# TuringLang/AdvancedHMC.jl

Hardware: AMD Instinct MI355X
Metric: leapfrog-steps/sec (whole node) at n_chains x D (higher is better)
Workload: dtype f64

## Files before the change

### advancedhmc.jl_amd/csrc/ahmc_device.hpp

```cpp
#pragma once

#include <hip/hip_runtime.h>
#include <stdint.h>

namespace ahmc {

enum : uint32_t { RNG_MOMENTUM = 0, RNG_TRANSITION = 1, RNG_JITTER = 2, RNG_FINDEPS = 3 };
constexpr uint32_t COUPLED_CHAIN = 0xFFFFFFFFu;

struct Philox4 {
  uint32_t v[4];
};

__device__ __forceinline__ Philox4 philox4x32_10(uint32_t c0, uint32_t c1, uint32_t c2, uint32_t c3,
                                                 uint32_t k0, uint32_t k1) {
  constexpr uint32_t M0 = 0xD2511F53u, M1 = 0xCD9E8D57u, W0 = 0x9E3779B9u, W1 = 0xBB67AE85u;
#pragma unroll
  for (int round = 0; round < 10; ++round) {
    uint32_t hi0 = __umulhi(M0, c0), lo0 = M0 * c0;
    uint32_t hi1 = __umulhi(M1, c2), lo1 = M1 * c2;
    uint32_t n0 = hi1 ^ c1 ^ k0, n2 = hi0 ^ c3 ^ k1;
    c0 = n0; c1 = lo1; c2 = n2; c3 = lo0;
    k0 += W0; k1 += W1;
  }
// ... 130 lines not shown
  q = q * t;
  return __builtin_ldexp(__builtin_fma(tj, q, tj), k >> 6);
  }
  {
  const double xh = x < -1100.0 ? -1100.0 : x;
  const double dn = __builtin_rint(xh * C(0x3ff71547652b82feULL));
  double t = __builtin_fma(dn, C(0xbfe62e42fefa39efULL), xh);
  t = __builtin_fma(dn, C(0xbc7abc9e3b39803fULL), t);
  double q = __builtin_fma(t, C(0x3e5ade156a5dcb37ULL), C(0x3e928af3fca7ab0cULL));
  q = fma3(t, q, C(0x3ec71dee623fde64ULL));
  q = fma3(t, q, C(0x3efa01997c89e6b0ULL));
  q = fma3(t, q, C(0x3f2a01a014761f6eULL));
  q = fma3(t, q, C(0x3f56c16c1852b7b0ULL));
  q = fma3(t, q, C(0x3f81111111122322ULL));
  q = fma3(t, q, C(0x3fa55555555502a1ULL));
  q = fma3(t, q, C(0x3fc5555555555511ULL));
  q = fma3(t, q, C(0x3fe000000000000bULL));
  q = __builtin_fma(t, q, 1.0);
  q = __builtin_fma(t, q, 1.0);
  double z = __builtin_ldexp(q, (int)dn);
  return z;
  }
}
template <bool UNIFORM>
__device__ __forceinline__ float leaf_weight_exp(float x) { return exp(x); }

template <class T, bool UNIFORM>
__device__ __forceinline__ T alpha_from_logweight(T lw) {
  const T w = leaf_weight_exp<UNIFORM>(lw > T(0) ? T(0) : lw);
  return w >= T(1) ? T(1) : w;
}

template <int LA, int LB>
__device__ __forceinline__ double leaf_weight_exp_pair(double x, bool odd) {
  constexpr auto C = [](unsigned long long bits) { return __builtin_bit_cast(double, bits); };
  const double xc = x < -1100.0 ? -1100.0 : x;
  const double dk = __builtin_rint(xc * 92.33248261689366);
  double t = __builtin_fma(dk, -0x1.62e42fef00000p-7, xc);
  t = __builtin_fma(dk, -0x1.473de6af278edp-40, t);
  const int k = (int)dk;
  const int ka = __builtin_amdgcn_readlane(k, LA), kb = __builtin_amdgcn_readlane(k, LB);
  const double tja = C(EXP2_64_BITS[ka & 63]), tjb = C(EXP2_64_BITS[kb & 63]);
  const double tj = odd ? tjb : tja;
  double q = __builtin_fma(t, 8.3333333333333332e-03, 4.1666666666666664e-02);
  q = fma3(t, q, 1.6666666666666666e-01);
  q = fma3(t, q, 0.5);
  q = fma3(t, q, 1.0);
  q = q * t;
  return __builtin_ldexp(__builtin_fma(tj, q, tj), k >> 6);
}
template <int LA, int LB>
__device__ __forceinline__ float leaf_weight_exp_pair(float x, bool) { return exp(x); }

template <class T> __device__ __forceinline__ T maxabs(T a, T b) { return fabs(a) > fabs(b) ? a : b; }

template <int CTRL> __device__ __forceinline__ int dpp_i32(int v) {
  return __builtin_amdgcn_mov_dpp(v, CTRL, 0xf, 0xf, true);
}
template <int CTRL> __device__ __forceinline__ float dpp_mov(float v) {
  return __int_as_float(dpp_i32<CTRL>(__float_as_int(v)));
}
template <int CTRL> __device__ __forceinline__ double dpp_mov(double v) {
  int lo = __double2loint(v), hi = __double2hiint(v);
  return __hiloint2double(dpp_i32<CTRL>(hi), dpp_i32<CTRL>(lo));
}
__device__ __forceinline__ float swz16(float v) {
  return __int_as_float(__builtin_amdgcn_ds_swizzle(__float_as_int(v), 0x401F));
}
__device__ __forceinline__ double swz16(double v) {
  int lo = __builtin_amdgcn_ds_swizzle(__double2loint(v), 0x401F);
  int hi = __builtin_amdgcn_ds_swizzle(__double2hiint(v), 0x401F);
  return __hiloint2double(hi, lo);
}
__device__ __forceinline__ float xor16_sum(float v) {
  auto p = __builtin_amdgcn_permlane16_swap(__float_as_int(v), __float_as_int(v), false, false);
  return __int_as_float(p[0]) + __int_as_float(p[1]);
}
__device__ __forceinline__ double xor16_sum(double v) {
  auto lo = __builtin_amdgcn_permlane16_swap(__double2loint(v), __double2loint(v), false, false);
  auto hi = __builtin_amdgcn_permlane16_swap(__double2hiint(v), __double2hiint(v), false, false);
  return __hiloint2double(hi[0], lo[0]) + __hiloint2double(hi[1], lo[1]);
}
__device__ __forceinline__ float xor32_sum(float v) {
  auto p = __builtin_amdgcn_permlane32_swap(__float_as_int(v), __float_as_int(v), false, false);
  return __int_as_float(p[0]) + __int_as_float(p[1]);
}
__device__ __forceinline__ double xor32_sum(double v) {
  auto lo = __builtin_amdgcn_permlane32_swap(__double2loint(v), __double2loint(v), false, false);
  auto hi = __builtin_amdgcn_permlane32_swap(__double2hiint(v), __double2hiint(v), false, false);
  return __hiloint2double(hi[0], lo[0]) + __hiloint2double(hi[1], lo[1]);
}

#ifndef AHMC_MFMA_REDUCE
#define AHMC_MFMA_REDUCE 0
#endif
template <class T> struct MfmaRed;
template <> struct MfmaRed<double> {
  typedef double acc_t __attribute__((ext_vector_type(4)));
  static __device__ __forceinline__ acc_t mma(double a, double b, acc_t c) { return __builtin_amdgcn_mfma_f64_16x16x4f64(a, b, c, 0, 0, 0); }
  static constexpr unsigned SEL = 8u;
  static constexpr int RA = 0, RB = 2;
};
template <> struct MfmaRed<float> {
  typedef float acc_t __attribute__((ext_vector_type(4)));
  static __device__ __forceinline__ acc_t mma(float a, float b, acc_t c) { return __builtin_amdgcn_mfma_f32_16x16x4f32(a, b, c, 0, 0, 0); }
  static constexpr unsigned SEL = 1u;
// ... 87 lines not shown
    return (__builtin_amdgcn_ballot_w64(x <= T(0)) & 3ull) != 0ull;
  }
}

template <int G, class T>
__device__ __forceinline__ void wave_allsum4(T& a, T& b, T& c, T& d) {
  static_assert(G == 16 || G == 32 || G == 64, "quad reduction needs whole 16-lane rows");
  const bool odd = (threadIdx.x & 1u) != 0, up = (threadIdx.x & 2u) != 0;
  const T x = (odd ? b : a) + dpp_mov<0xB1>(odd ? a : b);
  const T y = (odd ? d : c) + dpp_mov<0xB1>(odd ? c : d);
  T z = (up ? y : x) + dpp_mov<0x4E>(up ? x : y);
  z += dpp_mov<0x124>(z);
  z += dpp_mov<0x128>(z);
  if constexpr (G >= 32) z = xor16_sum(z);
  if constexpr (G >= 64) z = xor32_sum(z);
  a = dpp_mov<0x150>(z);
  b = dpp_mov<0x151>(z);
  c = dpp_mov<0x152>(z);
  d = dpp_mov<0x153>(z);
}

#ifndef AHMC_PAIR_RED_QUAD
#define AHMC_PAIR_RED_QUAD 1
#endif
template <class T, int Q = AHMC_PAIR_RED_QUAD>
__device__ __forceinline__ bool wave64_pair_reduce(T da, T db, T& ea, T& eb) {
  static_assert(Q >= 0 && Q <= 3, "a row has four quads");
  const bool odd = (threadIdx.x & 1u) != 0, up = (threadIdx.x & 2u) != 0;
  const T x = (odd ? db : da) + dpp_mov<0xB1>(odd ? da : db);
  const T y = (odd ? eb : ea) + dpp_mov<0xB1>(odd ? ea : eb);
  T z = (up ? y : x) + dpp_mov<0x4E>(up ? x : y);
  z += dpp_mov<0x124>(z);
  z += dpp_mov<0x128>(z);
  z = xor16_sum(z);
  z = xor32_sum(z);
  const bool le0 = (__builtin_amdgcn_ballot_w64(z <= T(0)) & 3ull) != 0ull;
  ea = dpp_mov<0x150 + 4 * Q + 2>(z);
  eb = dpp_mov<0x150 + 4 * Q + 3>(z);
  return le0;
}
template <class T>
__device__ __forceinline__ bool wave64_pair_reduce_t(T da, T db, T ea, T eb, T& z) {
  const bool odd = (threadIdx.x & 1u) != 0, up = (threadIdx.x & 2u) != 0;
  const T x = (odd ? db : da) + dpp_mov<0xB1>(odd ? da : db);
  const T y = (odd ? eb : ea) + dpp_mov<0xB1>(odd ? ea : eb);
  z = (up ? y : x) + dpp_mov<0x4E>(up ? x : y);
  z += dpp_mov<0x124>(z);
  z += dpp_mov<0x128>(z);
  z = xor16_sum(z);
  z = xor32_sum(z);
  return (__builtin_amdgcn_ballot_w64(z <= T(0)) & 3ull) != 0ull;
}

template <int G, class T, int K>
__device__ __forceinline__ void wave_allsum(T (&v)[K]) {
  static_assert(G == 1 || G == 2 || G == 4 || G == 8 || G == 16 || G == 32 || G == 64, "bad group size");
  if constexpr (G >= 16 && K == 4) {
    wave_allsum4<G>(v[0], v[1], v[2], v[3]);
    return;
  }
  if constexpr (G >= 16 && K % 2 == 0) {
#pragma unroll
    for (int k = 0; k < K; k += 2) wave_allsum2<G>(v[k], v[k + 1]);
    return;
  }
  if constexpr (G >= 2) {
#pragma unroll
    for (int k = 0; k < K; ++k) v[k] += dpp_mov<0xB1>(v[k]);
  }
  if constexpr (G >= 4) {
#pragma unroll
    for (int k = 0; k < K; ++k) v[k] += dpp_mov<0x4E>(v[k]);
  }
  if constexpr (G >= 8) {
#pragma unroll
    for (int k = 0; k < K; ++k) v[k] += dpp_mov<0x141>(v[k]);
  }
  if constexpr (G >= 16) {
#pragma unroll
    for (int k = 0; k < K; ++k) v[k] += dpp_mov<0x140>(v[k]);
  }
  if constexpr (G >= 32) {
#pragma unroll
    for (int k = 0; k < K; ++k) {
      if constexpr ((AHMC_DS_REDUCE & 1) != 0) v[k] += ds_swz<SWZ_XOR16>(v[k]); else v[k] = xor16_sum(v[k]);
    }
  }
  if constexpr (G >= 64) {
#pragma unroll
    for (int k = 0; k < K; ++k) {
      if constexpr ((AHMC_DS_REDUCE & 1) != 0) v[k] += ds_xor32(v[k]); else v[k] = xor32_sum(v[k]);
    }
  }
}
__device__ __forceinline__ double* xwave_buf() {
  __shared__ __attribute__((aligned(16))) double buf[8 * 8];
  return buf;
}

template <int G, class T, int K>
__device__ __forceinline__ void group_allsum(T (&v)[K]) {
  if constexpr (G <= 64) {
    wave_allsum<G>(v);
  } else {
    static_assert(G == 128 || G == 256 || G == 512, "bad multi-wave group size");
    static_assert(K <= 8, "at most 8 values per reduction");
// ... 327 lines not shown
#pragma unroll
  for (int e = 0; e < E; ++e) z.r[e] = leapfrog_kick(z.r[e], eh, z.g[e]);
#pragma unroll
  for (int e = 0; e < E; ++e) z.th[e] = leapfrog_drift(z.th[e], eps, minv[e], z.r[e]);
  const T part = target_eval<T, G, E, TK>(tp, z.th, z.g, lane, d0);
#pragma unroll
  for (int e = 0; e < E; ++e) z.r[e] = leapfrog_kick(z.r[e], eh, z.g[e]);
  const T kin = kinetic_partial(z.r, minv);
  return part - kin / 2;
}
template <class T>
__device__ __forceinline__ T neg_energy_sanitized(T s) { return is_finite(s) ? s : -Lim<T>::inf(); }

template <int L> __device__ __forceinline__ float readlane_t(float v) { return __int_as_float(__builtin_amdgcn_readlane(__float_as_int(v), L)); }
template <int L> __device__ __forceinline__ double readlane_t(double v) {
  return __hiloint2double(__builtin_amdgcn_readlane(__double2hiint(v), L), __builtin_amdgcn_readlane(__double2loint(v), L));
}

template <class T> struct PairLeafStats {
  T w[2], sa[2], dH[2];
  bool redo[2], div[2];
};
template <class T, bool LINW, int Q = AHMC_PAIR_RED_QUAD>
__device__ __forceinline__ void pair_leaf_stats(T z, T H0, T delta_max, T lw_limit, PairLeafStats<T>& o) {
  static_assert(Q >= 0 && Q <= 3, "a row has four quads");
  constexpr int LA = 4 * Q + 2, LB = 4 * Q + 3;
  const bool odd = (threadIdx.x & 1u) != 0;
  const T ne = neg_energy_sanitized(dpp_mov<0xEE>(z));
  const T dH = -ne - H0;
  const T lw = H0 + ne;
  T w, sa;
  if constexpr (LINW) {
    w = leaf_weight_exp_pair<LA, LB>(lw, odd);
    sa = w >= T(1) ? T(1) : w;
  } else {
    const T wa = leaf_weight_exp_pair<LA, LB>(lw > T(0) ? T(0) : lw, odd);
    sa = wa >= T(1) ? T(1) : wa;
    w = lw;
  }
  const unsigned long long m_redo = __builtin_amdgcn_ballot_w64(lw > lw_limit);
  const unsigned long long m_div = __builtin_amdgcn_ballot_w64(!(-H0 < delta_max + ne));
  o.w[0] = readlane_t<LA>(w);
  o.w[1] = readlane_t<LB>(w);
  o.sa[0] = readlane_t<LA>(sa);
  o.sa[1] = readlane_t<LB>(sa);
  o.dH[0] = readlane_t<LA>(dH);
  o.dH[1] = readlane_t<LB>(dH);
  o.redo[0] = LINW && ((m_redo >> LA) & 1ull) != 0ull;
  o.redo[1] = LINW && ((m_redo >> LB) & 1ull) != 0ull;
  o.div[0] = ((m_div >> LA) & 1ull) != 0ull;
  o.div[1] = ((m_div >> LB) & 1ull) != 0ull;
}

template <class T, int G, int E, int TK, class F>
__device__ __forceinline__ void leapfrog_step_plus2(Point<T, E>& z, const T (&minv)[E], T eps, const TargetP<T>& tp, int lane, int d0,
                                                    T (&extra)[2], F&& partials, bool use_pre = false) {
  const T eh = eps / 2;
#pragma unroll
  for (int e = 0; e < E; ++e) z.r[e] = leapfrog_kick(z.r[e], eh, z.g[e]);
#pragma unroll
  for (int e = 0; e < E; ++e) z.th[e] = leapfrog_drift(z.th[e], eps, minv[e], z.r[e]);
  T red[4];
  red[0] = target_eval<T, G, E, TK>(tp, z.th, z.g, lane, d0, use_pre);
#pragma unroll
  for (int e = 0; e < E; ++e) z.r[e] = leapfrog_kick(z.r[e], eh, z.g[e]);
  red[1] = kinetic_partial(z.r, minv);
  partials(red[2], red[3]);
  hier_publish_next<T, G, E, TK>(z, minv, eps);
  leapfrog_allsum<G, TK>(red);
  z.lp = sanitize(red[0]);
  z.lk = sanitize(-red[1] / 2);
  extra[0] = red[2];
  extra[1] = red[3];
}

template <class T, int G, int E, int TK>
__device__ __forceinline__ void fill_caches(Point<T, E>& z, const T (&minv)[E], const TargetP<T>& tp, int lane, int d0) {
  T red[2];
  red[0] = target_eval<T, G, E, TK>(tp, z.th, z.g, lane, d0);
  red[1] = kinetic_partial(z.r, minv);
  leapfrog_allsum<G, TK>(red);
  z.lp = sanitize(red[0]);
  z.lk = sanitize(-red[1] / 2);
}

template <class T, int E, bool SB = false>
__device__ __forceinline__ void load_vec(T (&v)[E], const T* __restrict__ base, int64_t off, int d0, int D, T pad) {
  constexpr int CH = (E * sizeof(T) >= 16) ? (int)(16 / sizeof(T)) : E;
  if constexpr (SB) {
    const T* sb = base + off;
    if (CH > 1 && d0 + E <= D && (reinterpret_cast<uintptr_t>(sb) % (CH * sizeof(T)) == 0)) {
      using V = T __attribute__((ext_vector_type(CH)));
      unsigned bv = (unsigned)d0 * (unsigned)sizeof(T);
      asm("; full lane" : "+v"(bv));
      const T* ptr = reinterpret_cast<const T*>(reinterpret_cast<const char*>(sb) + bv);
#pragma unroll
      for (int e = 0; e < E; e += CH) {
        V t = *reinterpret_cast<const V*>(ptr + e);
#pragma unroll
        for (int k = 0; k < CH; ++k) v[e + k] = t[k];
      }
    } else {
#pragma unroll
      for (int e = 0; e < E; ++e) {
        v[e] = pad;
        if (d0 + e < D) {
// ... 69 lines not shown
```

### advancedhmc.jl_amd/csrc/ahmc_nuts.hpp

```cpp
#pragma once

#ifndef AHMC_LEAF_PROF
#define AHMC_LEAF_PROF 0
#endif
#if AHMC_LEAF_PROF
#undef AHMC_WAVE_TIMELINE
#define AHMC_WAVE_TIMELINE 1
#define AHMC_TL_WORDS 24
#define AHMC_LP_TICK(i) { __builtin_amdgcn_sched_barrier(0); const unsigned n_ = (unsigned)__builtin_amdgcn_readfirstlane((int)(unsigned)__builtin_readcyclecounter()); __builtin_amdgcn_sched_barrier(0); lp_t[i] += n_ - lp_c; lp_c = n_; }
#define AHMC_LP_COUNT(i, n) { lp_t[i] += (unsigned)(n); }
#else
#define AHMC_LP_TICK(i)
#define AHMC_LP_COUNT(i, n)
#endif
#ifndef AHMC_WAVE_TIMELINE
#define AHMC_WAVE_TIMELINE 0
#endif
#ifndef AHMC_TL_WORDS
#define AHMC_TL_WORDS 8
#endif

#include <type_traits>

#include "ahmc_kernels.hpp"



namespace ahmc {

template <bool ON, class P>
__device__ __forceinline__ const P* args_reread() {
  if constexpr (ON) {
    auto k = __builtin_amdgcn_kernarg_segment_ptr();
    asm volatile("" : "+s"(k));
    return (const P*)k;
  } else {
    return nullptr;
  }
}
template <bool ON, class P>
__device__ __forceinline__ const P& args_at(const P& p, const P* q) {
  if constexpr (ON) return *q;
  else return p;
}

template <bool ON, class A, class P>
__device__ __forceinline__ auto adapt_block_at(const A* ak, const P* args) {
  if constexpr (ON) return (const __attribute__((address_space(4))) A*)args->adaptk;
  else return ak;
}
template <bool ON, class Q>
__device__ __forceinline__ Q* as_global(Q* q) {
  if constexpr (ON) return (Q*)(__attribute__((address_space(1))) Q*)q;
  else return q;
}

__device__ __forceinline__ int64_t wave_scalar64(int64_t x) {
  const uint32_t lo = (uint32_t)__builtin_amdgcn_readfirstlane((int)(uint32_t)x), hi = (uint32_t)__builtin_amdgcn_readfirstlane((int)(uint32_t)((uint64_t)x >> 32));
  return (int64_t)(((uint64_t)hi << 32) | lo);
}

constexpr double LINW_LIMIT = 600.0;
enum { SL_OTH_TH = 0, SL_OTH_R = 1, SL_OTH_G = 2, SL_TREE_A = 3, SL_Z0_R = 4, SL_Z0_G = 5, SL_START_R = 6 };

template <class T, int E>
struct Chunking {
  static constexpr int CH = (E * sizeof(T) >= 16) ? (int)(16 / sizeof(T)) : E;
  static constexpr int NCH = E / CH;
};

#define AHMC_AS_LDS __attribute__((address_space(3)))
#define AHMC_AS_GLB __attribute__((address_space(1)))
template <class T, int E>
struct Slots {
  AHMC_AS_LDS T* lds;
  AHMC_AS_GLB T* glb;
  int n_lds;
  unsigned lane_off;

#define AHMC_SLOT_PUT(AS)                                                                                   \
  static __device__ __forceinline__ void put(AS T* __restrict__ sb, unsigned off, const T (&v)[E]) {         \
    constexpr int CH = Chunking<T, E>::CH, NCH = Chunking<T, E>::NCH;                                       \
    if constexpr (CH > 1) {                                                                                 \
      using V = T __attribute__((ext_vector_type(CH)));                                                     \
      _Pragma("unroll") for (int c = 0; c < NCH; ++c) {                                                     \
        V t;                                                                                                \
        _Pragma("unroll") for (int k = 0; k < CH; ++k) t[k] = v[c * CH + k];                                \
        *(AS V*)(&sb[off + (unsigned)(c * 64 * CH)]) = t;                                                    \
      }                                                                                                     \
    } else {                                                                                                \
      _Pragma("unroll") for (int c = 0; c < NCH; ++c) sb[off + (unsigned)(c * 64)] = v[c];                  \
    }                                                                                                       \
  }                                                                                                         \
  static __device__ __forceinline__ void get(const AS T* __restrict__ sb, unsigned off, T (&v)[E]) {         \
    constexpr int CH = Chunking<T, E>::CH, NCH = Chunking<T, E>::NCH;                                       \
    if constexpr (CH > 1) {                                                                                 \
      using V = T __attribute__((ext_vector_type(CH)));                                                     \
      _Pragma("unroll") for (int c = 0; c < NCH; ++c) {                                                     \
        V t = *(const AS V*)(&sb[off + (unsigned)(c * 64 * CH)]);                                            \
        _Pragma("unroll") for (int k = 0; k < CH; ++k) v[c * CH + k] = t[k];                                \
      }                                                                                                     \
    } else {                                                                                                \
      _Pragma("unroll") for (int c = 0; c < NCH; ++c) v[c] = sb[off + (unsigned)(c * 64)];                  \
    }                                                                                                       \
  }
  AHMC_SLOT_PUT(AHMC_AS_LDS)
  AHMC_SLOT_PUT(AHMC_AS_GLB)
#undef AHMC_SLOT_PUT
  __device__ __forceinline__ void store(int slot, const T (&v)[E]) const {
    constexpr int SE = Chunking<T, E>::NCH * 64 * Chunking<T, E>::CH;
    if (slot < n_lds) put(lds + slot * SE, lane_off, v);
    else put(glb + (size_t)(slot - n_lds) * SE, lane_off, v);
  }
  __device__ __forceinline__ void load(int slot, T (&v)[E]) const {
    constexpr int SE = Chunking<T, E>::NCH * 64 * Chunking<T, E>::CH;
    if (slot < n_lds) get(lds + slot * SE, lane_off, v);
    else get(glb + (size_t)(slot - n_lds) * SE, lane_off, v);
  }
  __device__ __forceinline__ void store_cold(int slot, unsigned extra, const T (&v)[E]) const {
    constexpr int SE = Chunking<T, E>::NCH * 64 * Chunking<T, E>::CH;
    put(glb + (size_t)(slot - n_lds) * SE, lane_off + extra, v);
  }
  __device__ __forceinline__ void load_cold(int slot, unsigned extra, T (&v)[E]) const {
    constexpr int SE = Chunking<T, E>::NCH * 64 * Chunking<T, E>::CH;
    get(glb + (size_t)(slot - n_lds) * SE, lane_off + extra, v);
  }
};

template <class T, int G, int E, int TK, bool TEMPER = true>
__device__ __forceinline__ void leapfrog_core(Point<T, E>& z, const T (&minv)[E], T eps, const TargetP<T>& tp,
                                              const LeapfrogP<T>& lf, int lane, int d0) {
  if constexpr (TEMPER) temper(lf, z.r, 1, true, 1);
  const T eh = eps / 2;
#pragma unroll
  for (int e = 0; e < E; ++e) z.r[e] = leapfrog_kick(z.r[e], eh, z.g[e]);
#pragma unroll
  for (int e = 0; e < E; ++e) z.th[e] = leapfrog_drift(z.th[e], eps, minv[e], z.r[e]);
  (void)target_eval<T, G, E, TK>(tp, z.th, z.g, lane, d0);
#pragma unroll
  for (int e = 0; e < E; ++e) z.r[e] = leapfrog_kick(z.r[e], eh, z.g[e]);
  if constexpr (TEMPER) temper(lf, z.r, 1, false, 1);
}

template <bool WIDE>
struct DrawStreamT {
  static constexpr uint32_t PERIOD = !WIDE ? 4u : 256u;
  Rng rng;
  uint32_t k;
  Philox4 blk;
  __device__ __forceinline__ uint32_t lane_block() const {
    if constexpr (!WIDE) return 0u;
    else return threadIdx.x & 63u;
  }
  __device__ __forceinline__ void init(const Rng& r) { rng = r; k = 0; }
  __device__ __forceinline__ void resume(const Rng& r, uint32_t k0) {
    rng = r;
    k = k0;
    if (k & (PERIOD - 1u)) blk = rng.raw(RNG_TRANSITION, ((k & ~(PERIOD - 1u)) >> 2) + lane_block());
  }
  __device__ __forceinline__ uint32_t word() {
    if ((k & (PERIOD - 1u)) == 0u) blk = rng.raw(RNG_TRANSITION, (k >> 2) + lane_block());
    const uint32_t lo = (k & 1u) ? blk.v[1] : blk.v[0], hi = (k & 1u) ? blk.v[3] : blk.v[2];
    uint32_t w = (k & 2u) ? hi : lo;
    if constexpr (WIDE) {
      const uint32_t ks = (uint32_t)__builtin_amdgcn_readfirstlane((int)k);
      const int src = (int)((ks >> 2) & 63u);
      w = (uint32_t)__builtin_amdgcn_readlane((int)w, src);
    }
    ++k;
    return w;
  }
  __device__ __forceinline__ double uniform() { return ((double)word() + 0.5) * 2.3283064365386962890625e-10; }
  __device__ __forceinline__ bool boolean() { return (word() >> 31) != 0; }
  __device__ __forceinline__ double randexp() { return -log(uniform()); }
};
typedef DrawStreamT<false> DrawStream;

template <class T, int G, int E, int MODE, int TK>
__global__ __launch_bounds__((G > 256 ? G : 256), (E >= 16 ? 1 : (MODE == 2 ? (E <= 2 ? 3 : 2) : (E <= 2 ? 4 : (E <= 4 ? 3 : 2))))) void k_nuts(KP<T> p) {
  constexpr int CPW = G >= 64 ? 1 : 64 / G;
  if constexpr (G == 64 && (MODE == 0 || MODE == 3)) {
    const unsigned int wave_id = blockIdx.x * (blockDim.x >> 6) + (threadIdx.x >> 6);
    if (wave_id >= p.n_chunks) {
      const unsigned int tw = (unsigned int)__builtin_amdgcn_readfirstlane((int)(wave_id - p.n_chunks));
      const int64_t rows = (int64_t)p.tail_n_trans * p.N, row0 = (int64_t)tw * p.tail_rows;
      if (tw < p.tail_waves && row0 < rows)
        normals_rows(p, p.tail_out, p.tail_iteration, (uint32_t)RNG_MOMENTUM, row0, row0 + p.tail_rows < rows ? row0 + p.tail_rows : rows, (int)(threadIdx.x & 63));
      return;
    }
  }
#define AHMC_UNI(b) (CPW == 1 ? (__builtin_amdgcn_ballot_w64(b) != 0) : (b))
#define AHMC_ANY(b) (CPW == 1 ? (bool)(b) : (__builtin_amdgcn_ballot_w64(b) != 0))
  constexpr int NCH = Chunking<T, E>::NCH, CH = Chunking<T, E>::CH;
  constexpr int SLOT_ELEMS = NCH * 64 * CH;
  extern __shared__ __attribute__((aligned(16))) unsigned char smem[];
  const int nwaves = blockDim.x >> 6;
  const int wib = threadIdx.x >> 6;
  const int lane64 = threadIdx.x & 63;
  int lane = (int)(threadIdx.x & (G - 1));
  int gi = G >= 64 ? 0 : lane64 / G;
  int d0 = lane * E;
  const int NLEV = p.max_depth > 1 ? p.max_depth - 1 : 1;
  constexpr bool LINW = MODE == 0 || MODE == 3;
  constexpr bool GENERAL = MODE == 2;
  constexpr bool FUSE_M0 = !GENERAL && G > 64;
  constexpr bool ADAPT = MODE >= 3;
  constexpr bool UTURN_ANY = G == 64;
  constexpr bool PAIR = G == 64 && !GENERAL && UTURN_ANY && !AHMC_MFMA_REDUCE && (AHMC_DS_REDUCE & 3) == 0 &&
                        !AHMC_LEAF_PROF && !AHMC_WAVE_TIMELINE;
  const bool strict = GENERAL && p.criterion == 2;
  const int NV = strict ? 3 : 2;
  const int n_slots = NV * NLEV + NUTS_DORMANT + NUTS_CKPT;
  const int CK0 = NV * NLEV + NUTS_DORMANT;
  const int n_lds_slots = p.n_lds_levels;
  T* lds_vec = reinterpret_cast<T*>(smem) + (size_t)wib * n_lds_slots * SLOT_ELEMS;
  T* sT = reinterpret_cast<T*>(smem) + (size_t)nwaves * n_lds_slots * SLOT_ELEMS + (size_t)wib * NUTS_NSC * NLEV * CPW;
  T* sAT = reinterpret_cast<T*>(smem) + (size_t)nwaves * (n_lds_slots * SLOT_ELEMS + NUTS_NSC * NLEV * CPW) + (size_t)wib * NUTS_NAT * CPW;
  int* sIbase = reinterpret_cast<int*>(reinterpret_cast<T*>(smem) + (size_t)nwaves * (n_lds_slots * SLOT_ELEMS + (NUTS_NSC * NLEV + NUTS_NAT) * CPW));
  int* sI = sIbase + (size_t)wib * NUTS_NSI * NLEV * CPW;
  int* sAI = sIbase + (size_t)nwaves * NUTS_NSI * NLEV * CPW + (size_t)wib * NUTS_NAI * CPW;
#define A_EPSNOM sAT[0 * CPW + gi]
#define A_DAEPS sAT[1 * CPW + gi]
#define A_DAMU sAT[2 * CPW + gi]
#define A_DAXBAR sAT[3 * CPW + gi]
#define A_DAHBAR sAT[4 * CPW + gi]
#define A_DAM sAI[0 * CPW + gi]
#define A_WVN sAI[1 * CPW + gi]
#define A_CHK sAI[2 * CPW + gi]
#define S_W(lvl) sT[((0) * NLEV + (lvl)) * CPW + gi]
#define S_CK(lvl) sI[((1) * NLEV + (lvl)) * CPW + gi]
  constexpr bool TSC = G == 64 && !GENERAL;
  const int64_t wave_slot = (int64_t)blockIdx.x * nwaves + wib;
  Slots<T, E> sl;
  sl.lds = (AHMC_AS_LDS T*)lds_vec;
  sl.glb = (AHMC_AS_GLB T*)(p.scratch + wave_slot * (int64_t)(n_slots - n_lds_slots) * SLOT_ELEMS);
  sl.n_lds = n_lds_slots;
  sl.lane_off = (unsigned)lane64 * CH;
  const int DORM = NV * NLEV;
  const int NL_HOT = NLEV < 4 ? NLEV : 4;
  const int HOT_END = 2 * NL_HOT - 1;
  const int COLD_DORM = HOT_END + 2 + 2 * (NLEV > 4 ? NLEV - 4 : 0);
  auto LA = [&](int l) -> int {
    if constexpr (GENERAL) return NV * l;
    else return l == 0 ? 0 : (l < NL_HOT ? 2 * l - 1 : HOT_END + 2 + 2 * (l - 4));
  };
  auto LRF = [&](int l) -> int {
    if constexpr (GENERAL) return NV * l + 1;
    else return l == 0 ? 0 : (l < NL_HOT ? 2 * l : HOT_END + 3 + 2 * (l - 4));
  };
  auto DS = [&](int k) -> int {
    if constexpr (GENERAL) return DORM + k;
    else return k == SL_TREE_A ? HOT_END : (k == SL_OTH_R ? HOT_END + 1
                : COLD_DORM + (k == SL_OTH_TH ? 0 : k == SL_OTH_G ? 1 : k == SL_Z0_R ? 2 : k == SL_Z0_G ? 3 : 4));
  };
  const bool classic = GENERAL && p.criterion == 0;
  const bool slice = GENERAL && p.sampler == 2;

  const unsigned int chunk = G > 64 ? blockIdx.x : blockIdx.x * nwaves + wib;
  if (chunk >= p.n_chunks) return;
  const int64_t slot = (int64_t)chunk * CPW + gi;
  const int64_t c = slot < p.N ? (p.order ? (int64_t)p.order[slot] : slot) : p.N;
  int64_t cc = c < p.N ? c : 0;
  if constexpr (TSC) cc = wave_scalar64(cc);
  const int kt0 = p.redo_only ? p.redo[cc] - 1 : 0;
  bool active = c < p.N && kt0 >= 0;
  if (!AHMC_ANY(active)) return;
  T minv[E];
  load_minv<T, E, TSC>(p, cc, d0, minv);
  T th_cur[E];
  load_vec<T, E, TSC>(th_cur, p.th(), cc * p.D, d0, p.D, T(0));
  const AdaptK<T>* ak0 = ADAPT ? static_cast<const AdaptK<T>*>(p.adaptk) : nullptr;
  const AdaptK<T>* ak = ak0;
  const KP<T>*pa_ = nullptr, *pe_ = nullptr;

  auto schedule = [&](int kt2, bool& do_push, bool& do_update, bool& wv_reset, bool& dareset) {
    do_push = do_update = wv_reset = dareset = false;
    if (ak->kind == AHMC_ADAPT_STAN) {
      const int64_t si = ak->stan_i0 + kt2 + 1;
      const bool in_window = si >= ak->window_start && si <= ak->window_end;
      bool window_end = false;
      for (int k2 = 0; k2 < ak->n_splits; ++k2) window_end = window_end || ak->splits[k2] == si;
      if (in_window && ak->has_mm) { do_push = true; do_update = window_end; }
      if (window_end) { dareset = true; wv_reset = ak->has_mm != 0; }
    } else if (ak->has_mm) {
      do_push = true;
      do_update = true;
    }
    if (ak->pooled) { do_update = false; wv_reset = false; }
// ... 76 lines not shown
      bool vleft = false;
      if (!done) vleft = AHMC_UNI(ds.boolean());
      const int v = vleft ? -1 : 1;
      const bool need_swap = AHMC_UNI(!done && (vleft != cur_is_left));
      if (AHMC_ANY(need_swap)) {
        if (need_swap) {
          if (jw > 0) {
            Point<T, E> t;
            sl.load(DS(SL_OTH_TH), t.th);
            sl.load(DS(SL_OTH_R), t.r);
            sl.load(DS(SL_OTH_G), t.g);
            sl.store(DS(SL_OTH_TH), cur.th);
            sl.store(DS(SL_OTH_R), cur.r);
            sl.store(DS(SL_OTH_G), cur.g);
            copy_vec(cur.th, t.th);
            copy_vec(cur.r, t.r);
            copy_vec(cur.g, t.g);
          }
          int ti = pos_cur; pos_cur = pos_oth; pos_oth = ti;
          cur_is_left = vleft;
        }
      }
      if (strict && AHMC_ANY(!done)) {
        if (!done) sl.store(DS(SL_START_R), cur.r);
      }
      if (CKPT && jw >= CKPT_MIN_JW) {
        bool ck_save = true;
        if constexpr (CPW == 1) ck_save = AHMC_UNI(!done && pos_cur != 0);
        if (ck_save) {
          const unsigned xo = (unsigned)(((A_CHK & 1) ^ 1) * 3 * SLOT_ELEMS);
          sl.store_cold(CK0 + 0, xo, cur.th);
          sl.store_cold(CK0 + 1, xo, cur.r);
          sl.store_cold(CK0 + 2, xo, cur.g);
        }
      }
      const uint32_t nleaf = 1u << jw;
      bool alive = !done;
      bool sub_term = false;
      T A_c[E], RF_c[E];
      T w_c = 0, sa_c = 0, dh_c = 0;
      int na_c = 0, ck_c = 0;
      AHMC_LP_TICK(5)
      for (uint32_t leaf = 1; leaf <= nleaf; ++leaf) {
        if (!AHMC_ANY(alive)) break;
        AHMC_LP_COUNT(8, 1)
#if AHMC_WAVE_TIMELINE
        tl_steps += 1;
        tl_alive += (unsigned long long)__builtin_popcountll(__builtin_amdgcn_ballot_w64(alive && lane == 0));
#endif
        bool pair = false;
        if constexpr (PAIR) {
          pair = jw > 0;
          if (pair) ++leaf;
        }
        const int nm = __builtin_ctz(leaf);
        T dots_m0[2] = {0, 0}, RF_m0[E];
        if (pair) {
          if constexpr (PAIR) {
            const T es = v > 0 ? eps : -eps;
            T ea = leapfrog_step_ne_partial<T, G, E, TK>(cur, minv, es, p.tp, lane, d0);
            T r_a[E];
            copy_vec(r_a, cur.r);
            T eb = leapfrog_step_ne_partial<T, G, E, TK>(cur, minv, es, p.tp, lane, d0);
            T dots[2] = {0, 0};
#pragma unroll
            for (int e = 0; e < E; ++e) {
              A_c[e] = r_a[e] + cur.r[e];
              dots[0] += A_c[e] * (minv[e] * r_a[e]);
              dots[1] += A_c[e] * (minv[e] * cur.r[e]);
            }
            T z_t;
            const bool turn_ab = wave64_pair_reduce_t(dots[0], dots[1], ea, eb, z_t);
            PairLeafStats<T> ps;
            pair_leaf_stats<T, LINW>(z_t, H0, p.delta_max, sizeof(T) == 4 ? T(60) : T(LINW_LIMIT), ps);
            auto leaf_apply = [&](const int i) {
              pos_cur += v;
              ck_c = pos_cur;
              w_c = ps.w[i];
              if constexpr (LINW) redo = redo || ps.redo[i];
              sub_term = ps.div[i];
              numerical = numerical || sub_term;
              sa_c = sa_c + ps.sa[i];
              na_c = na_c + 1;
              if (v > 0) { dh_c = maxabs(dh_c, ps.dH[i]); asm volatile(""); }
              else { dh_c = maxabs(ps.dH[i], dh_c); asm volatile(""); }
            };
            leaf_apply(0);
            if (!sub_term) {
              const T w_p = w_c;
              const int ck_p = ck_c;
              leaf_apply(1);
              if (!sub_term) {
                T w_new;
                if constexpr (LINW) w_new = w_p + w_c; else w_new = logaddexp(w_p, w_c);
                bool keep_first;
                if constexpr (LINW) keep_first = AHMC_UNI((T)ds.uniform() * w_new < w_p); else keep_first = AHMC_UNI(w_new < w_p + (T)ds.randexp());
                if (keep_first) ck_c = ck_p;
                w_c = w_new;
                sub_term = turn_ab;
                copy_vec(RF_c, r_a);
                AHMC_LP_COUNT(9, 1)
              }
            }
          }
        } else if (alive) {
          T ne_leaf = 0;
          if constexpr (GENERAL) {
            leapfrog_step<T, G, E, TK, true>(cur, minv, v > 0 ? eps : -eps, p.tp, p.lf, lane, d0, 1, 1);
          } else if (FUSE_M0 && nm > 0) {
            leapfrog_step_plus2<T, G, E, TK>(cur, minv, v > 0 ? eps : -eps, p.tp, lane, d0, dots_m0, [&](T& s0, T& s1) {
              T A_p[E];
              sl.load(LA(0), A_p);
              copy_vec(RF_m0, A_p);
              s0 = 0;
              s1 = 0;
#pragma unroll
              for (int e = 0; e < E; ++e) {
                A_c[e] = A_p[e] + cur.r[e];
                s0 += A_c[e] * (minv[e] * RF_m0[e]);
                s1 += A_c[e] * (minv[e] * cur.r[e]);
              }
            }, leaf > 1);
          } else if constexpr (G > 64) {
            leapfrog_step<T, G, E, TK, false>(cur, minv, v > 0 ? eps : -eps, p.tp, p.lf, lane, d0, 1, 1, leaf > 1);
            ne_leaf = cur.lp + cur.lk;
          } else {
#if AHMC_LEAF_PROF
            {
              const T e_ = v > 0 ? eps : -eps, eh_ = e_ / 2;
#pragma unroll
              for (int e = 0; e < E; ++e) cur.r[e] = leapfrog_kick(cur.r[e], eh_, cur.g[e]);
#pragma unroll
              for (int e = 0; e < E; ++e) cur.th[e] = leapfrog_drift(cur.th[e], e_, minv[e], cur.r[e]);
              const T part_ = target_eval<T, G, E, TK>(p.tp, cur.th, cur.g, lane, d0);
#pragma unroll
              for (int e = 0; e < E; ++e) cur.r[e] = leapfrog_kick(cur.r[e], eh_, cur.g[e]);
              const T kin_ = kinetic_partial(cur.r, minv);
              T sv_[1] = {part_ - kin_ / 2};
              asm volatile("" : "+v"(sv_[0]));
              AHMC_LP_TICK(0)
              leapfrog_allsum<G, TK>(sv_);
              asm volatile("" : "+v"(sv_[0]));
              AHMC_LP_TICK(1)
              ne_leaf = is_finite(sv_[0]) ? sv_[0] : -Lim<T>::inf();
            }
#else
            ne_leaf = leapfrog_step_ne<T, G, E, TK>(cur, minv, v > 0 ? eps : -eps, p.tp, lane, d0);
#endif
          }
#if AHMC_LEAF_PROF
          if (GENERAL || G > 64) AHMC_LP_TICK(0)
#endif
          pos_cur += v;
          const T ne = (GENERAL || (FUSE_M0 && nm > 0)) ? cur.lp + cur.lk : ne_leaf;
// ... 61 lines not shown
                A_c[e] = A_p[e];
              }
              group_allsum<G>(dots);
              sub_term = (dots[0] >= 0) || (dots[1] >= 0);
            } else if (!strict) {
              T dots[2] = {dots_m0[0], dots_m0[1]};
              if constexpr (!pre.value) {
                dots[0] = 0;
                dots[1] = 0;
#pragma unroll
                for (int e = 0; e < E; ++e) {
                  A_c[e] = A_p[e] + A_in[e];
                  dots[0] += A_c[e] * (minv[e] * RF_p[e]);
                  dots[1] += A_c[e] * (minv[e] * cur.r[e]);
                }
                if constexpr (!UTURN_ANY) group_allsum<G>(dots);
              }
              if constexpr (UTURN_ANY && !pre.value) sub_term = wave64_any_le0_pair(dots[0], dots[1]);
              else sub_term = AHMC_UNI(dots[0] <= 0) || AHMC_UNI(dots[1] <= 0);
            } else {
              T RL_p[E];
              sl.load(NV * lvl + 2, RL_p);
              T dots[6] = {0, 0, 0, 0, 0, 0};
#pragma unroll
              for (int e = 0; e < E; ++e) {
                const T rho = A_p[e] + A_in[e];
                const T rho2 = A_p[e] + RF_in[e];
                const T rho3 = RL_p[e] + A_in[e];
                dots[0] += rho * (minv[e] * RF_p[e]);
                dots[1] += rho * (minv[e] * cur.r[e]);
                dots[2] += rho2 * (minv[e] * RF_p[e]);
                dots[3] += rho2 * (minv[e] * RF_in[e]);
                dots[4] += rho3 * (minv[e] * RL_p[e]);
                dots[5] += rho3 * (minv[e] * cur.r[e]);
                A_c[e] = rho;
              }
              group_allsum<G>(dots);
              sub_term = (dots[0] <= 0) || (dots[1] <= 0) || (dots[2] <= 0) || (dots[3] <= 0) || (dots[4] <= 0) || (dots[5] <= 0);
            }
            if constexpr (pre.value) copy_vec(RF_c, RF_m0); else copy_vec(RF_c, RF_p);
            AHMC_LP_COUNT(9, 1)
          }
        };
        if constexpr (GENERAL) {
          for (int lvl = 0; lvl < nm; ++lvl) {
            const bool m = AHMC_UNI(alive && !sub_term);
            if (!AHMC_ANY(m)) break;
            if (m) merge_level(lvl, A_c, RF_c, std::false_type{});
          }
        } else if (nm > 0) {
          bool m = AHMC_UNI(alive && !sub_term);
          if (AHMC_ANY(m)) {
            if (m && !pair) merge_level(0, cur.r, cur.r, std::bool_constant<FUSE_M0>{});
            for (int lvl = 1; lvl < nm; ++lvl) {
              m = AHMC_UNI(alive && !sub_term);
              if (!AHMC_ANY(m)) break;
              if (m) merge_level(lvl, A_c, RF_c, std::false_type{});
            }
          }
        }
        AHMC_LP_TICK(3)
        if (alive && sub_term) {
          alive = false;
        } else if (alive && leaf < nleaf) {
          if (GENERAL || nm > 0) {
            sl.store(LA(nm), A_c);
            sl.store(LRF(nm), RF_c);
          } else {
            sl.store(LA(0), cur.r);
          }
          if (strict) sl.store(NV * nm + 2, cur.r);
          S_W(nm) = w_c;
          S_CK(nm) = ck_c;
        }
        AHMC_LP_TICK(4)
      }
      if constexpr (!GENERAL) {
        if (jw == 0) {
          copy_vec(A_c, cur.r);
          copy_vec(RF_c, cur.r);
        }
      }
      if (!done) {
        if (!sub_term) {
          ++depth;
          bool acc;
          if (slice) acc = w_tree * (T)ds.uniform() < w_c;
          else if constexpr (LINW) acc = AHMC_UNI((T)ds.uniform() * w_tree < w_c);
          else acc = AHMC_UNI(w_tree < w_c + (T)ds.randexp());
          if (acc) {
            ck_tree = ck_c;
            if constexpr (CKPT) {
              const int start = pos_cur - v * (int)nleaf;
              int chk = A_CHK;
              if (jw >= CKPT_MIN_JW && start != 0) chk = (start << 1) | ((chk & 1) ^ 1);
              else if (((chk >> 1) > 0) != (v > 0) || (chk >> 1) == 0) chk = chk & 1;
              A_CHK = chk;
            }
          }
        }
        sa_tree = sa_tree + sa_c;
        na_tree = na_tree + na_c;
        dh_tree = v < 0 ? maxabs(dh_c, dh_tree) : maxabs(dh_tree, dh_c);
        if constexpr (LINW) w_tree = w_tree + w_c; else w_tree = slice ? w_tree + w_c : logaddexp(w_tree, w_c);
        bool turn;
        T oth_r[E];
        sl.load(DS(SL_OTH_R), oth_r);
// ... 238 lines not shown
```

Baseline: 3.637 billion.

## Batch four NUTS leaves per iteration with a fused quad wave reduction

When the tree depth allows it, four leapfrog leaves are now processed per loop iteration instead of two. The two pair-level U-turn checks, the level-1 U-turn check and the four energies are all combined in one wave-wide DPP reduction, and the leaf weights come from a single quad exp evaluation. The level-1 merge therefore skips the generic merge_level path. The intent is to amortise reduction and control overhead across more leaves. Separately, the slot scratch base pointer is forced into scalar registers via readfirstlane and asm constraints, at the cost of more code, more register pressure and extra work when the chain would have terminated early.

```diff
diff --git a/advancedhmc.jl_amd/csrc/ahmc_device.hpp b/advancedhmc.jl_amd/csrc/ahmc_device.hpp
--- a/advancedhmc.jl_amd/csrc/ahmc_device.hpp
+++ b/advancedhmc.jl_amd/csrc/ahmc_device.hpp
@@ -206,6 +206,30 @@
 template <int LA, int LB>
 __device__ __forceinline__ float leaf_weight_exp_pair(float x, bool) { return exp(x); }
 
+template <int L0>
+__device__ __forceinline__ double leaf_weight_exp_quad(double x, bool odd, bool up) {
+  constexpr auto C = [](unsigned long long bits) { return __builtin_bit_cast(double, bits); };
+  const double xc = x < -1100.0 ? -1100.0 : x;
+  const double dk = __builtin_rint(xc * 92.33248261689366);
+  double t = __builtin_fma(dk, -0x1.62e42fef00000p-7, xc);
+  t = __builtin_fma(dk, -0x1.473de6af278edp-40, t);
+  const int k = (int)dk;
+  const int k0 = __builtin_amdgcn_readlane(k, L0), k1 = __builtin_amdgcn_readlane(k, L0 + 1);
+  const int k2 = __builtin_amdgcn_readlane(k, L0 + 2), k3 = __builtin_amdgcn_readlane(k, L0 + 3);
+  const double tj0 = C(EXP2_64_BITS[k0 & 63]), tj1 = C(EXP2_64_BITS[k1 & 63]);
+  const double tj2 = C(EXP2_64_BITS[k2 & 63]), tj3 = C(EXP2_64_BITS[k3 & 63]);
+  const double tjl = odd ? tj1 : tj0, tjh = odd ? tj3 : tj2;
+  const double tj = up ? tjh : tjl;
+  double q = __builtin_fma(t, 8.3333333333333332e-03, 4.1666666666666664e-02);
+  q = fma3(t, q, 1.6666666666666666e-01);
+  q = fma3(t, q, 0.5);
+  q = fma3(t, q, 1.0);
+  q = q * t;
+  return __builtin_ldexp(__builtin_fma(tj, q, tj), k >> 6);
+}
+template <int L0>
+__device__ __forceinline__ float leaf_weight_exp_quad(float x, bool, bool) { return exp(x); }
+
 template <class T> __device__ __forceinline__ T maxabs(T a, T b) { return fabs(a) > fabs(b) ? a : b; }
 
 template <int CTRL> __device__ __forceinline__ int dpp_i32(int v) {
@@ -399,6 +423,26 @@
   return (__builtin_amdgcn_ballot_w64(z <= T(0)) & 3ull) != 0ull;
 }
 
+template <class T>
+__device__ __forceinline__ T wave64_quad_pair(T a, T b) {
+  const bool odd = (threadIdx.x & 1u) != 0;
+  return (odd ? b : a) + dpp_mov<0xB1>(odd ? a : b);
+}
+template <class T>
+__device__ __forceinline__ unsigned long long wave64_quad_reduce_t(T xab, T xcd, T xl, T yab, T ycd, T& w) {
+  const bool up = (threadIdx.x & 2u) != 0, oq = (threadIdx.x & 4u) != 0, hq = (threadIdx.x & 8u) != 0;
+  const T rd = (up ? xcd : xab) + dpp_mov<0x4E>(up ? xab : xcd);
+  const T re = (up ? ycd : yab) + dpp_mov<0x4E>(up ? yab : ycd);
+  const T rl = xl + dpp_mov<0x4E>(xl);
+  const T z = (oq ? re : rd) + dpp_mov<0x124>(oq ? rd : re);
+  const T zl = rl + dpp_mov<0x124>(rl);
+  w = (hq ? zl : z) + dpp_mov<0x128>(hq ? z : zl);
+  w = xor16_sum(w);
+  w = xor32_sum(w);
+  return __builtin_amdgcn_ballot_w64(w <= T(0));
+}
+constexpr unsigned long long QUAD_TURN_AB = 0x3ull, QUAD_TURN_CD = 0xCull, QUAD_TURN_L1 = 0x300ull;
+
 template <int G, class T, int K>
 __device__ __forceinline__ void wave_allsum(T (&v)[K]) {
   static_assert(G == 1 || G == 2 || G == 4 || G == 8 || G == 16 || G == 32 || G == 64, "bad group size");
@@ -832,6 +876,44 @@
   o.div[1] = ((m_div >> LB) & 1ull) != 0ull;
 }
 
+__device__ __forceinline__ float readlane_at(float v, int l) { return __int_as_float(__builtin_amdgcn_readlane(__float_as_int(v), l)); }
+__device__ __forceinline__ double readlane_at(double v, int l) {
+  return __hiloint2double(__builtin_amdgcn_readlane(__double2hiint(v), l), __builtin_amdgcn_readlane(__double2loint(v), l));
+}
+template <class T> struct QuadLeafStats {
+  static constexpr int L0 = 4;
+  T w_l, sa_l, dH_l;
+  unsigned long long m_redo, m_div;
+  __device__ __forceinline__ T w(int k) const { return readlane_at(w_l, L0 + k); }
+  __device__ __forceinline__ T sa(int k) const { return readlane_at(sa_l, L0 + k); }
+  __device__ __forceinline__ T dH(int k) const { return readlane_at(dH_l, L0 + k); }
+  __device__ __forceinline__ bool redo(int k) const { return ((m_redo >> (L0 + k)) & 1ull) != 0ull; }
+  __device__ __forceinline__ bool div(int k) const { return ((m_div >> (L0 + k)) & 1ull) != 0ull; }
+};
+template <class T, bool LINW>
+__device__ __forceinline__ void quad_leaf_stats(T wz, T H0, T delta_max, T lw_limit, QuadLeafStats<T>& o) {
+  constexpr int L0 = QuadLeafStats<T>::L0;
+  const bool odd = (threadIdx.x & 1u) != 0, up = (threadIdx.x & 2u) != 0, oq = (threadIdx.x & 4u) != 0;
+  const T from_prev = dpp_mov<0x124>(wz);
+  const T ne = neg_energy_sanitized(oq ? wz : from_prev);
+  const T dH = -ne - H0;
+  const T lw = H0 + ne;
+  T w, sa;
+  if constexpr (LINW) {
+    w = leaf_weight_exp_quad<L0>(lw, odd, up);
+    sa = w >= T(1) ? T(1) : w;
+  } else {
+    const T wa = leaf_weight_exp_quad<L0>(lw > T(0) ? T(0) : lw, odd, up);
+    sa = wa >= T(1) ? T(1) : wa;
+    w = lw;
+  }
+  o.m_redo = LINW ? __builtin_amdgcn_ballot_w64(lw > lw_limit) : 0ull;
+  o.m_div = __builtin_amdgcn_ballot_w64(!(-H0 < delta_max + ne));
+  o.w_l = w;
+  o.sa_l = sa;
+  o.dH_l = dH;
+}
+
 template <class T, int G, int E, int TK, class F>
 __device__ __forceinline__ void leapfrog_step_plus2(Point<T, E>& z, const T (&minv)[E], T eps, const TargetP<T>& tp, int lane, int d0,
                                                     T (&extra)[2], F&& partials, bool use_pre = false) {
diff --git a/advancedhmc.jl_amd/csrc/ahmc_nuts.hpp b/advancedhmc.jl_amd/csrc/ahmc_nuts.hpp
--- a/advancedhmc.jl_amd/csrc/ahmc_nuts.hpp
+++ b/advancedhmc.jl_amd/csrc/ahmc_nuts.hpp
@@ -71,7 +71,7 @@
 
 #define AHMC_AS_LDS __attribute__((address_space(3)))
 #define AHMC_AS_GLB __attribute__((address_space(1)))
-template <class T, int E>
+template <class T, int E, bool SC = false>
 struct Slots {
   AHMC_AS_LDS T* lds;
   AHMC_AS_GLB T* glb;
@@ -109,13 +109,39 @@
 #undef AHMC_SLOT_PUT
   __device__ __forceinline__ void store(int slot, const T (&v)[E]) const {
     constexpr int SE = Chunking<T, E>::NCH * 64 * Chunking<T, E>::CH;
-    if (slot < n_lds) put(lds + slot * SE, lane_off, v);
-    else put(glb + (size_t)(slot - n_lds) * SE, lane_off, v);
+    if constexpr (SC) {
+      int nl = n_lds;
+      AHMC_AS_GLB T* gb = glb;
+      asm volatile("" : "+s"(nl), "+s"(gb));
+      if (slot < nl) {
+        put(lds + slot * SE, lane_off, v);
+      } else {
+        unsigned lo = lane_off;
+        asm volatile("" : "+v"(lo));
+        put(gb + (size_t)(slot - nl) * SE, lo, v);
+      }
+    } else {
+      if (slot < n_lds) put(lds + slot * SE, lane_off, v);
+      else put(glb + (size_t)(slot - n_lds) * SE, lane_off, v);
+    }
   }
   __device__ __forceinline__ void load(int slot, T (&v)[E]) const {
     constexpr int SE = Chunking<T, E>::NCH * 64 * Chunking<T, E>::CH;
-    if (slot < n_lds) get(lds + slot * SE, lane_off, v);
-    else get(glb + (size_t)(slot - n_lds) * SE, lane_off, v);
+    if constexpr (SC) {
+      int nl = n_lds;
+      AHMC_AS_GLB T* gb = glb;
+      asm volatile("" : "+s"(nl), "+s"(gb));
+      if (slot < nl) {
+        get(lds + slot * SE, lane_off, v);
+      } else {
+        unsigned lo = lane_off;
+        asm volatile("" : "+v"(lo));
+        get(gb + (size_t)(slot - nl) * SE, lo, v);
+      }
+    } else {
+      if (slot < n_lds) get(lds + slot * SE, lane_off, v);
+      else get(glb + (size_t)(slot - n_lds) * SE, lane_off, v);
+    }
   }
   __device__ __forceinline__ void store_cold(int slot, unsigned extra, const T (&v)[E]) const {
     constexpr int SE = Chunking<T, E>::NCH * 64 * Chunking<T, E>::CH;
@@ -175,6 +201,9 @@
   __device__ __forceinline__ double randexp() { return -log(uniform()); }
 };
 typedef DrawStreamT<false> DrawStream;
+
+template <class T, int E, int MODE>
+constexpr bool nuts_quad_step() { return true; }
 
 template <class T, int G, int E, int MODE, int TK>
 __global__ __launch_bounds__((G > 256 ? G : 256), (E >= 16 ? 1 : (MODE == 2 ? (E <= 2 ? 3 : 2) : (E <= 2 ? 4 : (E <= 4 ? 3 : 2))))) void k_nuts(KP<T> p) {
@@ -208,6 +237,7 @@
   constexpr bool UTURN_ANY = G == 64;
   constexpr bool PAIR = G == 64 && !GENERAL && UTURN_ANY && !AHMC_MFMA_REDUCE && (AHMC_DS_REDUCE & 3) == 0 &&
                         !AHMC_LEAF_PROF && !AHMC_WAVE_TIMELINE;
+  constexpr bool QUAD = PAIR && nuts_quad_step<T, E, MODE>();
   const bool strict = GENERAL && p.criterion == 2;
   const int NV = strict ? 3 : 2;
   const int n_slots = NV * NLEV + NUTS_DORMANT + NUTS_CKPT;
@@ -231,9 +261,10 @@
 #define S_CK(lvl) sI[((1) * NLEV + (lvl)) * CPW + gi]
   constexpr bool TSC = G == 64 && !GENERAL;
   const int64_t wave_slot = (int64_t)blockIdx.x * nwaves + wib;
-  Slots<T, E> sl;
+  Slots<T, E, QUAD> sl;
   sl.lds = (AHMC_AS_LDS T*)lds_vec;
-  sl.glb = (AHMC_AS_GLB T*)(p.scratch + wave_slot * (int64_t)(n_slots - n_lds_slots) * SLOT_ELEMS);
+  if constexpr (QUAD) sl.glb = (AHMC_AS_GLB T*)(p.scratch + wave_scalar64(wave_slot) * (int64_t)(n_slots - n_lds_slots) * SLOT_ELEMS);
+  else sl.glb = (AHMC_AS_GLB T*)(p.scratch + wave_slot * (int64_t)(n_slots - n_lds_slots) * SLOT_ELEMS);
   sl.n_lds = n_lds_slots;
   sl.lane_off = (unsigned)lane64 * CH;
   const int DORM = NV * NLEV;
@@ -416,54 +447,129 @@
         if constexpr (PAIR) {
           pair = jw > 0;
           if (pair) ++leaf;
+          if constexpr (QUAD) {
+            if (jw > 1) leaf += 2;
+          }
         }
         const int nm = __builtin_ctz(leaf);
         T dots_m0[2] = {0, 0}, RF_m0[E];
         if (pair) {
           if constexpr (PAIR) {
-            const T es = v > 0 ? eps : -eps;
-            T ea = leapfrog_step_ne_partial<T, G, E, TK>(cur, minv, es, p.tp, lane, d0);
-            T r_a[E];
-            copy_vec(r_a, cur.r);
-            T eb = leapfrog_step_ne_partial<T, G, E, TK>(cur, minv, es, p.tp, lane, d0);
-            T dots[2] = {0, 0};
-#pragma unroll
-            for (int e = 0; e < E; ++e) {
-              A_c[e] = r_a[e] + cur.r[e];
-              dots[0] += A_c[e] * (minv[e] * r_a[e]);
-              dots[1] += A_c[e] * (minv[e] * cur.r[e]);
-            }
-            T z_t;
-            const bool turn_ab = wave64_pair_reduce_t(dots[0], dots[1], ea, eb, z_t);
-            PairLeafStats<T> ps;
-            pair_leaf_stats<T, LINW>(z_t, H0, p.delta_max, sizeof(T) == 4 ? T(60) : T(LINW_LIMIT), ps);
-            auto leaf_apply = [&](const int i) {
-              pos_cur += v;
-              ck_c = pos_cur;
-              w_c = ps.w[i];
-              if constexpr (LINW) redo = redo || ps.redo[i];
-              sub_term = ps.div[i];
-              numerical = numerical || sub_term;
-              sa_c = sa_c + ps.sa[i];
-              na_c = na_c + 1;
-              if (v > 0) { dh_c = maxabs(dh_c, ps.dH[i]); asm volatile(""); }
-              else { dh_c = maxabs(ps.dH[i], dh_c); asm volatile(""); }
-            };
-            leaf_apply(0);
-            if (!sub_term) {
-              const T w_p = w_c;
-              const int ck_p = ck_c;
-              leaf_apply(1);
-              if (!sub_term) {
+            if (QUAD && jw > 1) {
+              const T es = v > 0 ? eps : -eps;
+              T dab[2] = {0, 0}, dcd[2] = {0, 0}, dl[2] = {0, 0};
+              const T e_a = leapfrog_step_ne_partial<T, G, E, TK>(cur, minv, es, p.tp, lane, d0);
+              copy_vec(RF_c, cur.r);
+              const T e_b = leapfrog_step_ne_partial<T, G, E, TK>(cur, minv, es, p.tp, lane, d0);
+#pragma unroll
+              for (int e = 0; e < E; ++e) {
+                A_c[e] = RF_c[e] + cur.r[e];
+                dab[0] += A_c[e] * (minv[e] * RF_c[e]);
+                dab[1] += A_c[e] * (minv[e] * cur.r[e]);
+              }
+              const T yab = wave64_quad_pair(e_a, e_b), xab = wave64_quad_pair(dab[0], dab[1]);
+              const T e_c = leapfrog_step_ne_partial<T, G, E, TK>(cur, minv, es, p.tp, lane, d0);
+              T r_c[E];
+              copy_vec(r_c, cur.r);
+              const T e_d = leapfrog_step_ne_partial<T, G, E, TK>(cur, minv, es, p.tp, lane, d0);
+#pragma unroll
+              for (int e = 0; e < E; ++e) {
+                const T rho_cd = r_c[e] + cur.r[e];
+                dcd[0] += rho_cd * (minv[e] * r_c[e]);
+                dcd[1] += rho_cd * (minv[e] * cur.r[e]);
+                A_c[e] = A_c[e] + rho_cd;
+                dl[0] += A_c[e] * (minv[e] * RF_c[e]);
+                dl[1] += A_c[e] * (minv[e] * cur.r[e]);
+              }
+              T w_t;
+              const unsigned long long turns =
+                  wave64_quad_reduce_t(xab, wave64_quad_pair(dcd[0], dcd[1]), wave64_quad_pair(dl[0], dl[1]), yab, wave64_quad_pair(e_c, e_d), w_t);
+              QuadLeafStats<T> qs;
+              quad_leaf_stats<T, LINW>(w_t, H0, p.delta_max, sizeof(T) == 4 ? T(60) : T(LINW_LIMIT), qs);
+              auto leaf_apply = [&](const int i) {
+                pos_cur += v;
+                ck_c = pos_cur;
+                w_c = qs.w(i);
+                if constexpr (LINW) redo = redo || qs.redo(i);
+                sub_term = qs.div(i);
+                numerical = numerical || sub_term;
+                sa_c = sa_c + qs.sa(i);
+                na_c = na_c + 1;
+                const T dH_i = qs.dH(i);
+                if (v > 0) { dh_c = maxabs(dh_c, dH_i); asm volatile(""); }
+                else { dh_c = maxabs(dH_i, dh_c); asm volatile(""); }
+              };
+              auto merge_apply = [&](const T w_p, const int ck_p, const bool turn) {
                 T w_new;
                 if constexpr (LINW) w_new = w_p + w_c; else w_new = logaddexp(w_p, w_c);
                 bool keep_first;
                 if constexpr (LINW) keep_first = AHMC_UNI((T)ds.uniform() * w_new < w_p); else keep_first = AHMC_UNI(w_new < w_p + (T)ds.randexp());
                 if (keep_first) ck_c = ck_p;
                 w_c = w_new;
-                sub_term = turn_ab;
-                copy_vec(RF_c, r_a);
+                sub_term = turn;
                 AHMC_LP_COUNT(9, 1)
+              };
+              auto pair_apply = [&](const int h, const bool turn) {
+                leaf_apply(2 * h);
+                if (!sub_term) {
+                  const T w_p = w_c;
+                  const int ck_p = ck_c;
+                  leaf_apply(2 * h + 1);
+                  if (!sub_term) merge_apply(w_p, ck_p, turn);
+                }
+              };
+              pair_apply(0, (turns & QUAD_TURN_AB) != 0ull);
+              if (!sub_term) {
+                const T w_ab = w_c;
+                const int ck_ab = ck_c;
+                pair_apply(1, (turns & QUAD_TURN_CD) != 0ull);
+                if (!sub_term) merge_apply(w_ab, ck_ab, (turns & QUAD_TURN_L1) != 0ull);
+              }
+            } else {
+              const T es = v > 0 ? eps : -eps;
+              T ea = leapfrog_step_ne_partial<T, G, E, TK>(cur, minv, es, p.tp, lane, d0);
+              T r_a[E];
+              copy_vec(r_a, cur.r);
+              T eb = leapfrog_step_ne_partial<T, G, E, TK>(cur, minv, es, p.tp, lane, d0);
+              T dots[2] = {0, 0};
+#pragma unroll
+              for (int e = 0; e < E; ++e) {
+                A_c[e] = r_a[e] + cur.r[e];
+                dots[0] += A_c[e] * (minv[e] * r_a[e]);
+                dots[1] += A_c[e] * (minv[e] * cur.r[e]);
+              }
+              T z_t;
+              const bool turn_ab = wave64_pair_reduce_t(dots[0], dots[1], ea, eb, z_t);
+              PairLeafStats<T> ps;
+              pair_leaf_stats<T, LINW>(z_t, H0, p.delta_max, sizeof(T) == 4 ? T(60) : T(LINW_LIMIT), ps);
+              auto leaf_apply = [&](const int i) {
+                pos_cur += v;
+                ck_c = pos_cur;
+                w_c = ps.w[i];
+                if constexpr (LINW) redo = redo || ps.redo[i];
+                sub_term = ps.div[i];
+                numerical = numerical || sub_term;
+                sa_c = sa_c + ps.sa[i];
+                na_c = na_c + 1;
+                if (v > 0) { dh_c = maxabs(dh_c, ps.dH[i]); asm volatile(""); }
+                else { dh_c = maxabs(ps.dH[i], dh_c); asm volatile(""); }
+              };
+              leaf_apply(0);
+              if (!sub_term) {
+                const T w_p = w_c;
+                const int ck_p = ck_c;
+                leaf_apply(1);
+                if (!sub_term) {
+                  T w_new;
+                  if constexpr (LINW) w_new = w_p + w_c; else w_new = logaddexp(w_p, w_c);
+                  bool keep_first;
+                  if constexpr (LINW) keep_first = AHMC_UNI((T)ds.uniform() * w_new < w_p); else keep_first = AHMC_UNI(w_new < w_p + (T)ds.randexp());
+                  if (keep_first) ck_c = ck_p;
+                  w_c = w_new;
+                  sub_term = turn_ab;
+                  copy_vec(RF_c, r_a);
+                  AHMC_LP_COUNT(9, 1)
+                }
               }
             }
           }
@@ -631,7 +737,7 @@
           bool m = AHMC_UNI(alive && !sub_term);
           if (AHMC_ANY(m)) {
             if (m && !pair) merge_level(0, cur.r, cur.r, std::bool_constant<FUSE_M0>{});
-            for (int lvl = 1; lvl < nm; ++lvl) {
+            for (int lvl = 1 + (QUAD && jw > 1 ? 1 : 0); lvl < nm; ++lvl) {
               m = AHMC_UNI(alive && !sub_term);
               if (!AHMC_ANY(m)) break;
               if (m) merge_level(lvl, A_c, RF_c, std::false_type{});
```

New measurement: 4.095 billion, median of 6. +12.6%, better.
